# zamazincode/cv-diffusion-model

Measured on AMD Instinct MI355X. Metric: images/sec (whole node), 256×256 4-step LCM 'small'; PSNR vs CPU ref, higher is better.
Workload: dtype fp16; 1 GPU; variant=small, 256x256, batch=32/GPU, 4 LCM steps, fp16, 1xMI355X (BASELINE configs[1] per GPU); global_batch=32, parallelism=single GPU

## Files before the change

### cv-diffusion-model_amd/csrc/irbx.hip

```cpp
#include <string>
#include <type_traits>
#include <vector>

#include "common.h"
#include "kernels.h"

namespace llie {

typedef uint32_t u32x2 __attribute__((ext_vector_type(2)));

typedef __bf16 bf16x2_t __attribute__((ext_vector_type(2)));
__device__ __forceinline__ float dot2_bf16(uint32_t a, uint32_t b, float c) {
  return __builtin_amdgcn_fdot2_f32_bf16(*reinterpret_cast<const bf16x2_t*>(&a), *reinterpret_cast<const bf16x2_t*>(&b), c, false);
}

template <typename T>
__device__ __forceinline__ typename Elem<T>::vec_t activate8(typename Elem<T>::vec_t v, const float* sc, const float* sh) {
  const u32x4 x = reinterpret_cast<const u32x4&>(v);
  const f32x4 s0 = *reinterpret_cast<const f32x4*>(sc), s1 = *reinterpret_cast<const f32x4*>(sc + 4);
  const f32x4 b0 = *reinterpret_cast<const f32x4*>(sh), b1 = *reinterpret_cast<const f32x4*>(sh + 4);
  u32x4 o;
  o[0] = act_clamp01_pack<T>(x[0], s0[0], s0[1], b0[0], b0[1]);
  o[1] = act_clamp01_pack<T>(x[1], s0[2], s0[3], b0[2], b0[3]);
  o[2] = act_clamp01_pack<T>(x[2], s1[0], s1[1], b1[0], b1[1]);
// ... 102 lines not shown
      if constexpr (POOL) {
#pragma unroll
        for (int gi = 0; gi < 2; ++gi) {
          left[gi] = gcol == 0; right[gi] = gcol == w16 - 1;
          top[gi] = gidx < w16; bot[gi] = gidx >= gbot;
          edge[gi] = left[gi] || right[gi] || top[gi] || bot[gi];
          ++gidx;
          gcol = gcol + 1 == w16 ? 0 : gcol + 1;
        }
      }
#pragma unroll
      for (int j = 0; j < NBW; ++j) {
        f32x16 acc;
#pragma unroll
        for (int r = 0; r < 16; ++r) acc[r] = 0.f;
#pragma unroll
        for (int s = 0; s < KS; ++s) acc = mfma16<T>(af[s], wf[j][s], acc);
        if constexpr (STAMP) {
          asm volatile("" ::"s"(__builtin_amdgcn_readfirstlane(__float_as_int(acc[15]))));
          stamp(3);
        }
        if constexpr (POOL) {
          constexpr uint32_t ones = PackedOne<T>::lo | PackedOne<T>::hi;
          uint32_t pk[8];
#pragma unroll
          for (int i = 0; i < 8; ++i) pk[i] = affine_clamp01_pack<T>(acc[2 * i], acc[2 * i + 1], sc2[j], sc2[j], sh2[j], sh2[j]);
          float gs[2];
#pragma unroll
          for (int gi = 0; gi < 2; ++gi) {
            gs[gi] = dot2_pk<T>(pk[4 * gi], ones, 0.f);
#pragma unroll
            for (int i = 1; i < 4; ++i) gs[gi] = dot2_pk<T>(pk[4 * gi + i], ones, gs[gi]);
            if (edge[gi]) {
              asm volatile("" ::: "memory");
              const uint32_t mc0 = (left[gi] && h == 0) ? PackedOne<T>::lo : 0u;
              const uint32_t mcw = (right[gi] && h == 1) ? PackedOne<T>::hi : 0u;
              c0s[j] = dot2_pk<T>(pk[4 * gi], mc0, c0s[j]);
              cws[j] = dot2_pk<T>(pk[4 * gi + 3], mcw, cws[j]);
              if (top[gi]) {
                r0s[j] += gs[gi];
                kk[j][0] = dot2_pk<T>(pk[4 * gi], mc0, kk[j][0]);
                kk[j][1] = dot2_pk<T>(pk[4 * gi + 3], mcw, kk[j][1]);
              }
              if (bot[gi]) {
                rhs[j] += gs[gi];
                kk[j][2] = dot2_pk<T>(pk[4 * gi], mc0, kk[j][2]);
                kk[j][3] = dot2_pk<T>(pk[4 * gi + 3], mcw, kk[j][3]);
              }
            }
          }
          s1[j] += gs[0] + gs[1];
          stamp(4);
          continue;
        }
        f32x2 t1 = {0.f, 0.f}, t2 = {0.f, 0.f};
#pragma unroll
        for (int r = 0; r < 16; r += 2) {
          const f32x2 v = {acc[r], acc[r + 1]};
          t1 += v;
          t2 = __builtin_elementwise_fma(v, v, t2);
        }
        s1[j] += t1[0] + t1[1];
        s2[j] += t2[0] + t2[1];
      }
    }
  }
  if constexpr (STAMP) {
    if (a.dbg && lane == 0) {
      const size_t wg = (size_t)blockIdx.z * gridDim.x + blockIdx.x;
      for (int i = 0; i < kXStamps; ++i) a.dbg[(wg * 4 + wave) * kXStamps + i] = i < 5 ? tk[i] : 0ull;
    }
  }
  const int ntiles = P / RP;
  if constexpr (POOL) {
#pragma unroll
    for (int j = 0; j < NBW; ++j) {
      float v[9] = {s1[j], r0s[j], rhs[j], c0s[j], cws[j], kk[j][0], kk[j][1], kk[j][2], kk[j][3]};
#pragma unroll
      for (int i = 0; i < 9; ++i) v[i] += __shfl_xor(v[i], 32, 64);
      if (h == 0) {
        const int c = (wave * NBW + j) * 32 + n;
        float t = 0.f;
#pragma unroll
        for (int tap = 0; tap < 9; ++tap) {
          const int ky = tap / 3, kx = tap % 3;
          float st = v[0];
          if (ky == 2) st -= v[1];
          if (ky == 0) st -= v[2];
          if (kx == 2) st -= v[3];
          if (kx == 0) st -= v[4];
          if (ky == 2 && kx == 2) st += v[5];
          if (ky == 2 && kx == 0) st += v[6];
          if (ky == 0 && kx == 2) st += v[7];
          if (ky == 0 && kx == 0) st += v[8];
          t = __builtin_fmaf((float)(T)(6.f * a.wd[tap * a.Chid + c]), st, t);
        }
        fixed_add(a.pool_tot + (size_t)b * a.Chid + c, t, kPoolFixScale);
      }
    }
    return;
  }
#pragma unroll
  for (int j = 0; j < NBW; ++j) {
    s1[j] += __shfl_xor(s1[j], 32, 64);
    s2[j] += __shfl_xor(s2[j], 32, 64);
    if (h == 0) {
      const int c = (wave * NBW + j) * 32 + n;
      a.stats[((size_t)(b * ntiles + tile) * 2 + 0) * a.Chid + c] = 6.f * s1[j];
      a.stats[((size_t)(b * ntiles + tile) * 2 + 1) * a.Chid + c] = 36.f * s2[j];
    }
  }
}
template <int KS, int NBW>
__global__ void __launch_bounds__(256, 2) expand_pool_stamp_kernel(const IrbxArgs a, const int RP) {
  expand_scan<half_t, KS, NBW, true, true>(a, RP);
}
template <typename T, int KS, int NBW>
__global__ void __launch_bounds__(256, 2) expand_stats_kernel(const IrbxArgs a, const int RP) {
  expand_scan<T, KS, NBW, false>(a, RP);
}
template <typename T, int KS, int NBW>
__global__ void __launch_bounds__(256, 2) expand_pool_kernel(const IrbxArgs a, const int RP) {
  expand_scan<T, KS, NBW, true>(a, RP);
}

constexpr int kXT_H = 8, kXT_W = 16;
constexpr int kXH_W = kXT_W + 2, kXH_H = kXT_H + 2;
constexpr int kXNPX = kXH_W * kXH_H;
constexpr int kXNPB = 6;

constexpr int SHP = 144;

template <typename T, int KS, bool DBUF, bool STAMP, bool NTST, int PCO>
__device__ __forceinline__ void expand_dw_body(const IrbxArgs& a, const int tiles_per_wg, const int chunks_per_wg) {
  constexpr int K = 16 * KS;
  constexpr int XP = (K + 8) * 2;
  constexpr int QSTEP = 256 / (2 * KS);
  constexpr int XTHR = QSTEP * 2 * KS;
  constexpr int XPT = (kXNPX + QSTEP - 1) / QSTEP;
  constexpr int SH_BYTES = kXNPB * 32 * SHP;
  constexpr bool PREF = KS <= 2;
  typedef typename Elem<T>::vec_t vec_t;
  extern __shared__ __align__(16) unsigned char smem[];
  unsigned char* sH = smem;
  unsigned char* sX = smem + (DBUF ? 2 : 1) * SH_BYTES;
  T* wds = reinterpret_cast<T*>(sX + kXNPB * 32 * XP);
  float* aff2 = reinterpret_cast<float*>(wds + 10 * a.Chid);
  float* aff1 = aff2 + 2 * a.Chid;
  float* red = aff1 + 2 * K;
  constexpr bool PACC_LDS = KS <= 4;
  long long* pacc_lds = reinterpret_cast<long long*>(red + 2 * 256);
  long long pacc_reg[PACC_LDS ? 1 : KS];
  constexpr bool PSKIP = PCO > 0 && PCO != K;
  float* gate_s = reinterpret_cast<float*>(red + (PSKIP ? 8 * PCO : 2 * 256));
  static_assert(PCO == 0 || (!DBUF && !STAMP && (PCO == K ? PACC_LDS : PCO % 32 == 0 && PCO <= 64)),
                "project tail: single-buffered kernel; identity blocks keep the gate in the pool totals' LDS");

  const int tid = threadIdx.x, lane = tid & 63, wave = tid >> 6;
  const int n = lane & 31, h = lane >> 5;
  const int chb = wave & 1, pxg = wave >> 1;
  const int b = blockIdx.z;
  const int tiles_x = a.W / kXT_W;
  const int P = a.H * a.W;
  const T* x0 = reinterpret_cast<const T*>(a.x0) + (size_t)b * P * a.c0;
  const T* x1 = a.x1 ? reinterpret_cast<const T*>(a.x1) + (size_t)b * P * a.c1 : nullptr;
  const T* w1 = reinterpret_cast<const T*>(a.w1);
  T* out = reinterpret_cast<T*>(a.out) + (size_t)b * P * a.Chid;
  const int chunk0 = blockIdx.y * chunks_per_wg;
  const int nchunks_all = a.Chid / 64;
  const int chunk1 = chunk0 + chunks_per_wg < nchunks_all ? chunk0 + chunks_per_wg : nchunks_all;

  for (int i = tid; i < 10 * a.Chid; i += 256) {
    const int t = i & 1, c = (i >> 1) % a.Chid, tap = 2 * ((i >> 1) / a.Chid) + t;
    wds[i] = tap < 9 ? (T)(6.f * a.wd[tap * a.Chid + c]) : (T)0.f;
  }
  for (int i = tid; i < a.Chid; i += 256) {
    aff2[i] = a.as2[(size_t)b * a.Chid + i];
    aff2[a.Chid + i] = a.ab2[(size_t)b * a.Chid + i] * kSixth;
  }
  for (int i = tid; i < K; i += 256) {
    aff1[i] = a.as1[(size_t)b * K + i];
    aff1[K + i] = a.ab1[(size_t)b * K + i];
  }
  if constexpr (PCO > 0)
    for (int i = tid; i < a.Chid; i += 256) gate_s[i] = a.gate[(size_t)b * a.Chid + i];
  for (int i = tid; i < (kXNPB * 32 - kXNPX) * (XP / 16); i += 256)
    *reinterpret_cast<u32x4*>(sX + kXNPX * XP + i * 16) = u32x4{0u, 0u, 0u, 0u};

  const int ntiles_img = tiles_x * (a.H / kXT_H);
  const int tile_first = tiles_per_wg > 0 ? blockIdx.x * tiles_per_wg : (int)(blockIdx.x * (unsigned)ntiles_img / gridDim.x);
  const int tile_end = tiles_per_wg > 0 ? tile_first + tiles_per_wg : (int)((blockIdx.x + 1) * (unsigned)ntiles_img / gridDim.x);
  const int tile_last = tile_end < ntiles_img ? tile_end : ntiles_img;

  const int xkv = tid % (2 * KS), xq0 = tid / (2 * KS), xk8 = xkv * 8;
  const bool xthr = XTHR == 256 || tid < XTHR;
  const bool xseg1 = xk8 >= a.c0;
  const T* xb = xseg1 ? x1 + (xk8 - a.c0) : x0 + xk8;
  const int xc = xseg1 ? a.c1 : a.c0;
  const bool xlast = xthr && (XPT - 1) * QSTEP + xq0 < kXNPX;
  int xrel[XPT];
#pragma unroll
  for (int j = 0; j < XPT; ++j) {
    const int q = xq0 + j * QSTEP;
    xrel[j] = (q / kXH_W - 1) * a.W + (q % kXH_W - 1);
  }
  unsigned char* sxw = sX + xq0 * XP + xk8 * 2;
  vec_t raw[XPT];
  auto load_tile = [&](int ty, int tx) {
    const int pix0 = ty * kXT_H * a.W + tx * kXT_W;
    const bool border = ty == 0 || tx == 0 || ty == a.H / kXT_H - 1 || tx == tiles_x - 1;
    if (!border) {
#pragma unroll
      for (int j = 0; j < XPT; ++j) {
        if (j < XPT - 1 ? xthr : xlast) raw[j] = ld_vec<T>(xb + (size_t)(pix0 + xrel[j]) * xc);
        else raw[j] = vec_t{};
      }
    } else {
#pragma unroll
      for (int j = 0; j < XPT; ++j) {
        const int q = xq0 + j * QSTEP;
        const int gy = ty * kXT_H - 1 + q / kXH_W, gx = tx * kXT_W - 1 + q % kXH_W;
        if ((j < XPT - 1 ? xthr : xlast) && gy >= 0 && gy < a.H && gx >= 0 && gx < a.W) raw[j] = ld_vec<T>(xb + (size_t)(pix0 + xrel[j]) * xc);
        else raw[j] = vec_t{};
      }
    }
  };
  int ty = tile_first / tiles_x, tx = tile_first % tiles_x;
  if (PREF && tile_first < tile_last) load_tile(ty, tx);
  vec_t wf[KS];
  auto load_wf = [&](int chunk) {
#pragma unroll
    for (int s = 0; s < KS; ++s) wf[s] = ld_vec<T>(w1 + (size_t)(chunk * 64 + chb * 32 + n) * K + 16 * s + 8 * h);
  };
  load_wf(chunk0);
  wg_barrier();

  unsigned long long tk[kXStamps] = {}, t_prev = 0;
  auto stamp = [&](int slot) {
    if constexpr (STAMP) {
      __builtin_amdgcn_sched_barrier(0);
      const unsigned long long now = __builtin_amdgcn_s_memtime();
      __builtin_amdgcn_sched_barrier(0);
      if (slot >= 0) tk[slot] += now - t_prev;
      t_prev = now;
    }
  };
  stamp(-1);
  const bool has_pool = PCO == 0 && (a.pool != nullptr || a.pool_tot != nullptr);
  int par = 0;
  int pend_tile = -1, pend_chunk = 0, pend_par = 0;
  if constexpr (PCO > 0) {
  } else if constexpr (PACC_LDS) {
    if (tid < 64) {
#pragma unroll
      for (int q = 0; q < KS; ++q) pacc_lds[q * 64 + tid] = 0;
    }
  } else {
#pragma unroll
    for (int q = 0; q < KS; ++q) pacc_reg[q] = 0;
  }
  auto flush_pool = [&]() {
    if constexpr (PCO > 0) {
      if (pend_tile >= 0 && tid < 2 * PCO) {
        const float t = (red[tid] + red[2 * PCO + tid]) + (red[4 * PCO + tid] + red[6 * PCO + tid]);
        a.ystats[((size_t)b * ntiles_img + pend_tile) * 2 * PCO + tid] = t;
      }
      pend_tile = -1;
      return;
    }
    if (pend_tile >= 0 && tid < 64) {
      const float* r = red + pend_par * 256;
      const int cbb = tid >> 5, ci = tid & 31;
      const float t = r[cbb * 64 + ci] + r[(cbb + 2) * 64 + ci];
      if (a.pool_tot) {
        const long long v = __float2ll_rn(t * kPoolFixScale);
        if constexpr (PACC_LDS) {
          pacc_lds[(pend_chunk - chunk0) * 64 + tid] += v;
        } else {
#pragma unroll
          for (int q = 0; q < KS; ++q) pacc_reg[q] += (pend_chunk - chunk0 == q) ? v : 0ll;
        }
      } else {
        a.pool[((size_t)b * ntiles_img + pend_tile) * a.Chid + pend_chunk * 64 + tid] = t;
      }
    }
    pend_tile = -1;
  };

  for (int tile = tile_first; tile < tile_last; ++tile) {
    const int y0 = ty * kXT_H, x0p = tx * kXT_W;
    int tyn = ty, txn = tx + 1;
    if (txn == tiles_x) { txn = 0; ++tyn; }
    if (!PREF) load_tile(ty, tx);
    __builtin_amdgcn_s_waitcnt(0x0F70);
    stamp(0);
#pragma unroll
    for (int j = 0; j < XPT; ++j) {
      if (j < XPT - 1 ? xthr : xlast)
        *reinterpret_cast<vec_t*>(sxw + j * QSTEP * XP) = activate8<T>(raw[j], aff1 + xk8, aff1 + K + xk8);
    }
    stamp(1);
    if (PREF && tile + 1 < tile_last) load_tile(tyn, txn);
    const bool border = ty == 0 || tx == 0 || ty == a.H / kXT_H - 1 || tx == tiles_x - 1;
    bool ok[3] = {true, true, true};
    if (border) {
#pragma unroll
      for (int i = 0; i < 3; ++i) {
        const int q = (pxg * 3 + i) * 32 + n;
        const int gy = y0 - 1 + q / kXH_W, gx = x0p - 1 + q % kXH_W;
        ok[i] = q < kXNPX && gy >= 0 && gy < a.H && gx >= 0 && gx < a.W;
      }
    }
    stamp(2);
    wg_barrier();
    stamp(3);
    if (!DBUF) flush_pool();
    stamp(4);

    typedef float f32x4v __attribute__((ext_vector_type(4)));
    constexpr int NCB = PCO > 0 ? PCO / 16 : 1;
    f32x4v yacc[2][NCB];
#pragma unroll
    for (int r = 0; r < 2; ++r)
#pragma unroll
      for (int cb = 0; cb < NCB; ++cb) yacc[r][cb] = f32x4v{0.f, 0.f, 0.f, 0.f};
    for (int chunk = chunk0; chunk < chunk1; ++chunk) {
      unsigned char* buf = sH + (DBUF ? par * SH_BYTES : 0);
      if (!DBUF && chunk > chunk0) {
        wg_barrier();
        flush_pool();
        stamp(5);
      }
      const int ch0 = chunk * 64 + chb * 32;
      f32x4 sc2[4], sh2[4];
#pragma unroll
      for (int g = 0; g < 4; ++g) {
        sc2[g] = *reinterpret_cast<const f32x4*>(aff2 + ch0 + 8 * g + 4 * h);
        sh2[g] = *reinterpret_cast<const f32x4*>(aff2 + a.Chid + ch0 + 8 * g + 4 * h);
      }
      constexpr int NACC = (KS <= 2 && PCO == 0) ? 3 : 1;
      f32x16 accs[NACC];
      if constexpr (NACC == 3) {
#pragma unroll
        for (int i = 0; i < 3; ++i) {
          const int q = (pxg * 3 + i) * 32 + n;
#pragma unroll
          for (int r = 0; r < 16; ++r) accs[i][r] = 0.f;
#pragma unroll
          for (int s = 0; s < KS; ++s)
            accs[i] = mfma16<T>(wf[s], *reinterpret_cast<const vec_t*>(sX + q * XP + (16 * s + 8 * h) * 2), accs[i]);
        }
        load_wf(chunk + 1 < chunk1 ? chunk + 1 : chunk0);
      }
#pragma unroll
      for (int i = 0; i < 3; ++i) {
        const int q = (pxg * 3 + i) * 32 + n;
        if constexpr (NACC == 1) {
#pragma unroll
          for (int r = 0; r < 16; ++r) accs[0][r] = 0.f;
#pragma unroll
          for (int s = 0; s < KS; ++s)
            accs[0] = mfma16<T>(wf[s], *reinterpret_cast<const vec_t*>(sX + q * XP + (16 * s + 8 * h) * 2), accs[0]);
          if (i == 2) load_wf(chunk + 1 < chunk1 ? chunk + 1 : chunk0);
        }
        const f32x16 acc = accs[NACC == 3 ? i : 0];
        uint32_t pk[4][2];
#pragma unroll
        for (int g = 0; g < 4; ++g)
#pragma unroll
          for (int j = 0; j < 2; ++j)
            pk[g][j] = affine_clamp01_pack<T>(acc[4 * g + 2 * j], acc[4 * g + 2 * j + 1], sc2[g][2 * j], sc2[g][2 * j + 1],
                                              sh2[g][2 * j], sh2[g][2 * j + 1]);
        if (border) {
#pragma unroll
          for (int g = 0; g < 4; ++g)
#pragma unroll
            for (int j = 0; j < 2; ++j) pk[g][j] = ok[i] ? pk[g][j] : 0u;
        }
        u32x4 lo, hi2;
#pragma unroll
        for (int j = 0; j < 2; ++j) {
          const u32x2 r02 = __builtin_amdgcn_permlane32_swap(pk[0][j], pk[2][j], false, false);
          const u32x2 r13 = __builtin_amdgcn_permlane32_swap(pk[1][j], pk[3][j], false, false);
          lo[j] = r02[0]; lo[2 + j] = r02[1];
          hi2[j] = r13[0]; hi2[2 + j] = r13[1];
        }
        *reinterpret_cast<u32x4*>(buf + q * SHP + (chb * 4 + 2 * h) * 16) = lo;
        *reinterpret_cast<u32x4*>(buf + q * SHP + (chb * 4 + 2 * h + 1) * 16) = hi2;
      }
      stamp(6);
      wg_barrier();
      if (DBUF) flush_pool();
      stamp(7);
      if constexpr (PCO > 0) {
        const int li = lane & 15, g = lane >> 4;
        uint32_t amask[4];
#pragma unroll
        for (int d = 0; d < 4; ++d)
          amask[d] = (((li & 7) >> 1) == d && (g >> 1) == (li >> 3)) ? ((li & 1) ? 0xFFFF0000u : 0x0000FFFFu) : 0u;
        const uint32_t* wpair = reinterpret_cast<const uint32_t*>(wds) + chunk * 64 + li;
        const uint32_t wsel = (g & 1) ? 0x03020302u : 0x01000100u;
        const int choff = 8 * (g >> 1) + 16 * (g & 1);
        vec_t wpf[NCB][2];
        const T* wp = reinterpret_cast<const T*>(a.wp) + (size_t)li * a.ldp + chunk * 64 + choff;
#pragma unroll
        for (int cb = 0; cb < NCB; ++cb)
#pragma unroll
          for (int kb = 0; kb < 2; ++kb) wpf[cb][kb] = ld_vec<T>(wp + (size_t)cb * 16 * a.ldp + 32 * kb);
        f32x4v dacc[4][2];
#pragma unroll
        for (int c = 0; c < 4; ++c)
#pragma unroll
          for (int r = 0; r < 2; ++r) dacc[c][r] = f32x4v{0.f, 0.f, 0.f, 0.f};
        const unsigned char* bbase = buf + ((2 * wave) * kXH_W + li) * SHP + (g >> 1) * 16;
        const bool upper = (g & 1) != 0;
        vec_t bf[2][2];
        uint32_t wq[2];
        auto ld_step = [&](int step, vec_t (&bb)[2], uint32_t& w2) {
          const int pr = step >> 2, c = step & 3;
          const int ta = 2 * pr, tb = 2 * pr + 1 < 9 ? 2 * pr + 1 : 8;
          const int offa = (ta / 3) * kXH_W + ta % 3, offb = (tb / 3) * kXH_W + tb % 3;
          const unsigned char* p0 = bbase + (upper ? offb : offa) * SHP + c * 32;
#pragma unroll
          for (int r = 0; r < 2; ++r) bb[r] = *reinterpret_cast<const vec_t*>(p0 + r * kXH_W * SHP);
          w2 = wpair[pr * a.Chid + 16 * c];
        };
        ld_step(0, bf[0], wq[0]);
#pragma unroll
        for (int step = 0; step < 20; ++step) {
          if (step + 1 < 20) ld_step(step + 1, bf[(step + 1) & 1], wq[(step + 1) & 1]);
          __builtin_amdgcn_sched_barrier(0);
          const int c = step & 3;
          const uint32_t wdup = __builtin_amdgcn_perm(wq[step & 1], wq[step & 1], wsel);
          u32x4 t;
#pragma unroll
          for (int d = 0; d < 4; ++d) t[d] = wdup & amask[d];
          const vec_t af = reinterpret_cast<const vec_t&>(t);
#pragma unroll
          for (int r = 0; r < 2; ++r) dacc[c][r] = mfma16x16<T>(af, bf[step & 1][r], dacc[c][r]);
        }
#pragma unroll
        for (int c = 0; c < 4; ++c) {
          const f32x4 gt = *reinterpret_cast<const f32x4*>(gate_s + chunk * 64 + 16 * c + 4 * g);
#pragma unroll
          for (int r = 0; r < 2; ++r)
#pragma unroll
            for (int e = 0; e < 4; ++e) dacc[c][r][e] *= gt[e];
        }
#pragma unroll
        for (int r = 0; r < 2; ++r)
#pragma unroll
          for (int kb = 0; kb < 2; ++kb) {
            uint32_t p0[2], p1[2];
#pragma unroll
            for (int j = 0; j < 2; ++j) {
              typedef T t2 __attribute__((ext_vector_type(2)));
              t2 o0, o1;
              o0[0] = (T)dacc[2 * kb][r][2 * j]; o0[1] = (T)dacc[2 * kb][r][2 * j + 1];
              o1[0] = (T)dacc[2 * kb + 1][r][2 * j]; o1[1] = (T)dacc[2 * kb + 1][r][2 * j + 1];
              p0[j] = *reinterpret_cast<uint32_t*>(&o0);
              p1[j] = *reinterpret_cast<uint32_t*>(&o1);
            }
            const u32x2 s0 = __builtin_amdgcn_permlane16_swap(p0[0], p1[0], false, false);
            const u32x2 s1 = __builtin_amdgcn_permlane16_swap(p0[1], p1[1], false, false);
            const u32x4 v = {s0[0], s1[0], s0[1], s1[1]};
#pragma unroll
            for (int cb = 0; cb < NCB; ++cb) yacc[r][cb] = mfma16x16<T>(wpf[cb][kb], reinterpret_cast<const vec_t&>(v), yacc[r][cb]);
          }
      } else {
        const int li = lane & 15, g = lane >> 4;
        uint32_t amask[4];
#pragma unroll
        for (int d = 0; d < 4; ++d)
          amask[d] = (((li & 7) >> 1) == d && (g >> 1) == (li >> 3)) ? ((li & 1) ? 0xFFFF0000u : 0x0000FFFFu) : 0u;
        const uint32_t* wpair = reinterpret_cast<const uint32_t*>(wds) + chunk * 64 + chb * 32 + li;
        const uint32_t wsel = (g & 1) ? 0x03020302u : 0x01000100u;
        f32x4v dacc[2][4];
#pragma unroll
        for (int c2 = 0; c2 < 2; ++c2)
#pragma unroll
          for (int r = 0; r < 4; ++r) dacc[c2][r] = f32x4v{0.f, 0.f, 0.f, 0.f};
        const unsigned char* bbase = buf + ((4 * pxg) * kXH_W + li) * SHP + (chb * 4 + (g >> 1)) * 16;
        const bool upper = (g & 1) != 0;
        vec_t bf[2][4];
        uint32_t wq[2];
        auto ld_step = [&](int step, vec_t (&bb)[4], uint32_t& w2) {
          const int pr = step >> 1, c2 = step & 1;
          const int ta = 2 * pr, tb = 2 * pr + 1 < 9 ? 2 * pr + 1 : 8;
          const int offa = (ta / 3) * kXH_W + ta % 3, offb = (tb / 3) * kXH_W + tb % 3;
          const unsigned char* p0 = bbase + (upper ? offb : offa) * SHP + c2 * 32;
#pragma unroll
          for (int r = 0; r < 4; ++r) bb[r] = *reinterpret_cast<const vec_t*>(p0 + r * kXH_W * SHP);
          w2 = wpair[pr * a.Chid + 16 * c2];
        };
        ld_step(0, bf[0], wq[0]);
#pragma unroll
        for (int step = 0; step < 10; ++step) {
          if (step + 1 < 10) ld_step(step + 1, bf[(step + 1) & 1], wq[(step + 1) & 1]);
          __builtin_amdgcn_sched_barrier(0);
          const int c2 = step & 1;
          const uint32_t wdup = __builtin_amdgcn_perm(wq[step & 1], wq[step & 1], wsel);
          u32x4 t;
#pragma unroll
          for (int d = 0; d < 4; ++d) t[d] = wdup & amask[d];
          const vec_t af = reinterpret_cast<const vec_t&>(t);
#pragma unroll
          for (int r = 0; r < 4; ++r) dacc[c2][r] = mfma16x16<T>(af, bf[step & 1][r], dacc[c2][r]);
        }
        const int choff = 8 * (g >> 1) + 16 * (g & 1);
#pragma unroll
        for (int r = 0; r < 4; ++r) {
          uint32_t p0[2], p1[2];
#pragma unroll
          for (int j = 0; j < 2; ++j) {
            typedef T t2 __attribute__((ext_vector_type(2)));
            t2 o0, o1;
            o0[0] = (T)dacc[0][r][2 * j]; o0[1] = (T)dacc[0][r][2 * j + 1];
            o1[0] = (T)dacc[1][r][2 * j]; o1[1] = (T)dacc[1][r][2 * j + 1];
            p0[j] = *reinterpret_cast<uint32_t*>(&o0);
            p1[j] = *reinterpret_cast<uint32_t*>(&o1);
          }
          const u32x2 s0 = __builtin_amdgcn_permlane16_swap(p0[0], p1[0], false, false);
          const u32x2 s1 = __builtin_amdgcn_permlane16_swap(p0[1], p1[1], false, false);
          const u32x4 v = {s0[0], s1[0], s0[1], s1[1]};
          const int orow = 4 * pxg + r;
          T* op = out + ((size_t)(y0 + orow) * a.W + x0p + li) * a.Chid + chunk * 64 + chb * 32 + choff;
          if constexpr (NTST) __builtin_nontemporal_store(v, reinterpret_cast<u32x4*>(op));
          else *reinterpret_cast<u32x4*>(op) = v;
        }
        if (has_pool) {
          float v[8];
#pragma unroll
          for (int c2 = 0; c2 < 2; ++c2)
#pragma unroll
            for (int e = 0; e < 4; ++e) v[4 * c2 + e] = (dacc[c2][0][e] + dacc[c2][1][e]) + (dacc[c2][2][e] + dacc[c2][3][e]);
#define LLIE_DPP_STEP(ROR)                                                                                               \
  _Pragma("unroll") for (int i = 0; i < 8; ++i)                                                                          \
      asm volatile("v_add_f32_dpp %0, %0, %0 row_ror:" #ROR " row_mask:0xf bank_mask:0xf" : "+v"(v[i]));
          asm volatile("s_nop 1" : "+v"(v[0]), "+v"(v[1]), "+v"(v[2]), "+v"(v[3]), "+v"(v[4]), "+v"(v[5]), "+v"(v[6]), "+v"(v[7]));
          LLIE_DPP_STEP(8)
          LLIE_DPP_STEP(4)
          LLIE_DPP_STEP(2)
          LLIE_DPP_STEP(1)
#undef LLIE_DPP_STEP
          if (li == 0) {
            float* rp = red + (DBUF ? par : 0) * 256 + wave * 64 + 4 * g;
            *reinterpret_cast<f32x4*>(rp) = f32x4{v[0], v[1], v[2], v[3]};
            *reinterpret_cast<f32x4*>(rp + 16) = f32x4{v[4], v[5], v[6], v[7]};
          }
          pend_tile = tile; pend_chunk = chunk; pend_par = DBUF ? par : 0;
        }
      }
      if (DBUF) par ^= 1;
      stamp(8);
    }
    if constexpr (PCO > 0) {
      const int li = lane & 15, g = lane >> 4;
      const int choff = 8 * (g >> 1) + 16 * (g & 1);
      T* yout = reinterpret_cast<T*>(a.y) + (size_t)b * P * PCO;
      if constexpr (PSKIP) {
        const T* wsk = reinterpret_cast<const T*>(a.wp) + (size_t)li * a.ldp + a.Chid + 8 * g;
#pragma unroll
        for (int ks = 0; ks < K / 32; ++ks) {
          const int ch = 32 * ks + 8 * g;
          vec_t wsf[NCB];
#pragma unroll
          for (int cb = 0; cb < NCB; ++cb) wsf[cb] = ld_vec<T>(wsk + (size_t)cb * 16 * a.ldp + 32 * ks);
#pragma unroll
          for (int r = 0; r < 2; ++r) {
            const size_t pix = (size_t)(y0 + 2 * wave + r) * a.W + x0p + li;
            const vec_t xv = ch < a.c0 ? ld_vec<T>(x0 + pix * a.c0 + ch) : ld_vec<T>(x1 + pix * a.c1 + (ch - a.c0));
#pragma unroll
            for (int cb = 0; cb < NCB; ++cb) yacc[r][cb] = mfma16x16<T>(wsf[cb], xv, yacc[r][cb]);
          }
        }
      }
      float st[2][NCB * 4];
#pragma unroll
      for (int i = 0; i < NCB * 4; ++i) st[0][i] = st[1][i] = 0.f;
#pragma unroll
      for (int r = 0; r < 2; ++r) {
        const size_t pix = (size_t)(y0 + 2 * wave + r) * a.W + x0p + li;
        uint32_t pk[NCB][2];
#pragma unroll
        for (int cb = 0; cb < NCB; ++cb) {
          typedef T t4 __attribute__((ext_vector_type(4)));
          typedef T t2 __attribute__((ext_vector_type(2)));
          t4 res = t4{};
          if constexpr (!PSKIP) res = *reinterpret_cast<const t4*>(x0 + pix * PCO + 16 * cb + 4 * g);
#pragma unroll
          for (int j = 0; j < 2; ++j) {
            t2 o;
#pragma unroll
            for (int e = 0; e < 2; ++e) {
              o[e] = PSKIP ? (T)yacc[r][cb][2 * j + e] : (T)(yacc[r][cb][2 * j + e] + (float)res[2 * j + e]);
              const float q = (float)o[e];
              st[0][4 * cb + 2 * j + e] += q;
              st[1][4 * cb + 2 * j + e] = __builtin_fmaf(q, q, st[1][4 * cb + 2 * j + e]);
            }
            pk[cb][j] = *reinterpret_cast<uint32_t*>(&o);
          }
        }
#pragma unroll
        for (int pp = 0; pp < NCB / 2; ++pp) {
          const u32x2 s0 = __builtin_amdgcn_permlane16_swap(pk[2 * pp][0], pk[2 * pp + 1][0], false, false);
          const u32x2 s1 = __builtin_amdgcn_permlane16_swap(pk[2 * pp][1], pk[2 * pp + 1][1], false, false);
          *reinterpret_cast<u32x4*>(yout + pix * PCO + 32 * pp + choff) = u32x4{s0[0], s1[0], s0[1], s1[1]};
        }
      }
#pragma unroll
      for (int w8 = 0; w8 < NCB; ++w8) {
        float* v = &st[w8 & 1][(w8 >> 1) * 8];
#define LLIE_DPP_STEP(ROR)                                                                                               \
  _Pragma("unroll") for (int i = 0; i < 8; ++i)                                                                          \
      asm volatile("v_add_f32_dpp %0, %0, %0 row_ror:" #ROR " row_mask:0xf bank_mask:0xf" : "+v"(v[i]));
        asm volatile("s_nop 1" : "+v"(v[0]), "+v"(v[1]), "+v"(v[2]), "+v"(v[3]), "+v"(v[4]), "+v"(v[5]), "+v"(v[6]), "+v"(v[7]));
        LLIE_DPP_STEP(8)
        LLIE_DPP_STEP(4)
        LLIE_DPP_STEP(2)
        LLIE_DPP_STEP(1)
#undef LLIE_DPP_STEP
      }
      if (li == 0) {
#pragma unroll
        for (int which = 0; which < 2; ++which)
#pragma unroll
          for (int cb = 0; cb < NCB; ++cb)
            *reinterpret_cast<f32x4*>(red + (wave * 2 + which) * PCO + 16 * cb + 4 * g) =
                f32x4{st[which][4 * cb], st[which][4 * cb + 1], st[which][4 * cb + 2], st[which][4 * cb + 3]};
      }
      pend_tile = tile;
    }
    ty = tyn; tx = txn;
  }
  if constexpr (STAMP) {
    if (a.dbg && lane == 0) {
      const size_t wg = ((size_t)blockIdx.z * gridDim.y + blockIdx.y) * gridDim.x + blockIdx.x;
#pragma unroll
      for (int i = 0; i < kXStamps; ++i) a.dbg[(wg * 4 + wave) * kXStamps + i] = tk[i];
    }
  }
  if constexpr (PCO > 0) {
    wg_barrier();
    flush_pool();
  }
  if (has_pool) {
    wg_barrier();
    flush_pool();
    if (a.pool_tot && tid < 64) {
#pragma unroll
      for (int q = 0; q < KS; ++q)
        if (chunk0 + q < chunk1) atomicAdd(a.pool_tot + (size_t)b * a.Chid + (chunk0 + q) * 64 + tid, (unsigned long long)(PACC_LDS ? pacc_lds[q * 64 + tid] : pacc_reg[PACC_LDS ? 0 : q]));
    }
  }
}

template <typename T, int KS, bool DBUF, bool STAMP = false, bool NTST = false>
__global__ void __launch_bounds__(256, (KS == 2 && !DBUF) ? 3 : 2) expand_dw_kernel(const IrbxArgs a, const int tiles_per_wg, const int chunks_per_wg) {
  expand_dw_body<T, KS, DBUF, STAMP, NTST, 0>(a, tiles_per_wg, chunks_per_wg);
}
template <typename T, int KS, int PCO>
__global__ void __launch_bounds__(256, KS == 2 ? 3 : 2) expand_dw_project_kernel(const IrbxArgs a, const int tiles_per_wg) {
  expand_dw_body<T, KS, false, false, false, PCO>(a, tiles_per_wg, KS);
}

bool irbx_supported(int dtype, int Cin, int c0, int Chid, int H, int W) {
  if (dtype != 1 && dtype != 2) return false;
  if (Cin != 32 && Cin != 64 && Cin != 96) return false;
  if (c0 % 16 || Chid != 4 * Cin) return false;
  return W % kXT_W == 0 && H % kXT_H == 0 && (H * W) % irbx_stats_rows(H * W) == 0;
}
int irbx_pool_tiles(int H, int W) { return (H / kXT_H) * (W / kXT_W); }
int irbx_project_supported(int dtype, int Cin, int c0, int Chid, int Cout, bool skip, int H, int W) {
  if (!irbx_supported(dtype, Cin, c0, Chid, H, W)) return 0;
  if (!skip) return (Cin == 32 || Cin == 64) && Cout == Cin && c0 == Cin ? kIrbxProjectIdentity : 0;
  return Cin == 96 && Cout == 32 ? kIrbxProjectSkip : 0;
}
int irbx_project_tiles(int H, int W) { return irbx_pool_tiles(H, W); }
int irbx_stats_rows(int P) {
  int rp = 128;
  while (rp < 1024 && rp * 2 * 64 <= P) rp *= 2;
  return rp;
}

static int g_irbx_dbuf = 0, g_irbx_stamp = 0;
static int g_irbx_grid[3] = {0, 0, 0};
void irbx_grid(int ks, int v) {
  for (int i = 0; i < 3; ++i)
    if (ks == 0 || ks == 2 * (i + 1)) g_irbx_grid[i] = v;
}
static unsigned long long* g_irbx_dbg = nullptr;
static size_t g_irbx_dbg_n = 0;
void irbx_stamp(int v) { g_irbx_stamp = v; }
hipError_t irbx_stamp_fetch(double* out) {
  if (!g_irbx_dbg || !g_irbx_dbg_n) return hipErrorInvalidValue;
  std::vector<unsigned long long> h(g_irbx_dbg_n);
  hipError_t e = hipMemcpy(h.data(), g_irbx_dbg, g_irbx_dbg_n * 8, hipMemcpyDeviceToHost);
  if (e != hipSuccess) return e;
  for (int i = 0; i < kXStamps; ++i) out[i] = 0.0;
  for (size_t i = 0; i < g_irbx_dbg_n; ++i) out[i % kXStamps] += (double)h[i];
  for (int i = 0; i < kXStamps; ++i) out[i] /= (double)(g_irbx_dbg_n / kXStamps);
  out[kXStamps] = (double)(g_irbx_dbg_n / kXStamps);
  return hipSuccess;
}
void irbx_tune(int dbuf) { if (dbuf >= 0) g_irbx_dbuf = dbuf; }

template <typename T, int KS, int NBW, bool POOL>
static hipError_t launch_scan_cfg(const IrbxArgs& a, hipStream_t s) {
  const int P = a.H * a.W, RP = irbx_stats_rows(P);
  static const std::string name = std::string(POOL ? "expand_pool_kernel<" : "expand_stats_kernel<") + TypeName<T>::value + ", " +
                                  std::to_string(KS) + ", " + std::to_string(NBW) + ">";
  note_kernel(name.c_str());
  if constexpr (POOL && std::is_same<T, half_t>::value) {
    if (g_irbx_stamp == 2) {
      IrbxArgs b = a;
      const size_t n = (size_t)(P / RP) * a.B * 4 * kXStamps;
      if (n > g_irbx_dbg_n || !g_irbx_dbg) {
        if (g_irbx_dbg) (void)hipFree(g_irbx_dbg);
        hipError_t e = hipMalloc(reinterpret_cast<void**>(&g_irbx_dbg), n * 8);
        if (e != hipSuccess) return e;
      }
      g_irbx_dbg_n = n;
      b.dbg = g_irbx_dbg;
      hipLaunchKernelGGL((expand_pool_stamp_kernel<KS, NBW>), dim3(P / RP, 1, a.B), dim3(256), 0, s, b, RP);
      return hipGetLastError();
    }
  }
  constexpr auto kernel = POOL ? &expand_pool_kernel<T, KS, NBW> : &expand_stats_kernel<T, KS, NBW>;
  hipLaunchKernelGGL(kernel, dim3(P / RP, 1, a.B), dim3(256), 0, s, a, RP);
  return hipGetLastError();
}
template <typename T, bool POOL>
static hipError_t launch_scan_t(const IrbxArgs& a, hipStream_t s) {
  switch (a.c0 + a.c1) {
    case 32: return launch_scan_cfg<T, 2, 1, POOL>(a, s);
    case 64: return launch_scan_cfg<T, 4, 2, POOL>(a, s);
    case 96: return launch_scan_cfg<T, 6, 3, POOL>(a, s);
  }
  return hipErrorInvalidValue;
}
hipError_t launch_expand_stats(int dtype, const IrbxArgs& a, hipStream_t s) {
  if (!irbx_supported(dtype, a.c0 + a.c1, a.c0, a.Chid, a.H, a.W) || (a.c1 && !a.x1) || !a.stats) return hipErrorInvalidValue;
  return dtype == 1 ? launch_scan_t<half_t, false>(a, s) : launch_scan_t<bf16_t, false>(a, s);
}
hipError_t launch_expand_pool(int dtype, const IrbxArgs& a, hipStream_t s) {
  if (!irbx_supported(dtype, a.c0 + a.c1, a.c0, a.Chid, a.H, a.W) || (a.c1 && !a.x1) || !a.pool_tot || !a.as2 || !a.ab2 || !a.wd)
    return hipErrorInvalidValue;
  return dtype == 1 ? launch_scan_t<half_t, true>(a, s) : launch_scan_t<bf16_t, true>(a, s);
}

constexpr size_t irbx_lds_bytes(int KS, int Chid, bool dbuf, int PCO) {
  const size_t body = (size_t)(dbuf ? 2 : 1) * kXNPB * 32 * SHP + (size_t)kXNPB * 32 * (16 * KS + 8) * 2 + (size_t)10 * Chid * 2 +
                      (size_t)2 * Chid * 4 + (size_t)2 * 16 * KS * 4;
  if (PCO != 0 && PCO != 16 * KS) return body + (size_t)8 * PCO * 4 + (size_t)Chid * 4;
  return body + 2 * 256 * 4 + (KS <= 4 ? (size_t)KS * 64 * 8 : 0);
}
static_assert(irbx_lds_bytes(6, 384, false, 32) == 81664 && irbx_lds_bytes(6, 384, false, 32) <= 80 * 1024, "expand_dw_project<6, 32>: two workgroups per CU");

constexpr int kXTilesPerWg = 4;
static int irbx_tiles_per_wg(const IrbxArgs& a) {
  int tpw = kXTilesPerWg;
  while (tpw > 1 && ((a.W / kXT_W) % tpw || (long)(irbx_pool_tiles(a.H, a.W) / tpw) * a.B < 2048)) tpw >>= 1;
  return tpw;
}

template <typename T, int KS, bool DBUF, bool STAMP, bool NTST>
static hipError_t launch_dw_one(const IrbxArgs& a, dim3 grid, size_t lds, int tpw, int cpw, hipStream_t s) {
  static std::atomic<uint64_t> attr_done{0};
  if (hipError_t e = ensure_max_lds(reinterpret_cast<const void*>(&expand_dw_kernel<T, KS, DBUF, STAMP, NTST>), 128 * 1024, attr_done); e != hipSuccess)
    return e;
  hipLaunchKernelGGL((expand_dw_kernel<T, KS, DBUF, STAMP, NTST>), grid, dim3(256), lds, s, a, tpw, cpw);
  return hipGetLastError();
}
template <typename T, int KS, bool DBUF>
static hipError_t launch_dw_cfg(const IrbxArgs& a, hipStream_t s) {
  const size_t lds = irbx_lds_bytes(KS, a.Chid, DBUF, 0);
  const int ntiles = irbx_pool_tiles(a.H, a.W), nchunks = a.Chid / 64;
  int tpw = irbx_tiles_per_wg(a);
  int cpw = nchunks;
  while (cpw > 1 && (long)(ntiles / tpw) * a.B * (nchunks / cpw) < 1024 && cpw % 2 == 0) cpw >>= 1;
  static const std::string name = std::string("expand_dw_kernel<") + TypeName<T>::value + ", " + std::to_string(KS) + ", " +
                                  (DBUF ? "1" : "0") + ">";
  note_kernel(name.c_str());
  dim3 grid(ntiles / tpw, nchunks / cpw, a.B);
  if (g_irbx_grid[KS / 2 - 1] > 0) {
    int gx = g_irbx_grid[KS / 2 - 1] / (a.B * (nchunks / cpw));
    gx = gx < 1 ? 1 : (gx > ntiles ? ntiles : gx);
    grid.x = gx;
    tpw = 0;
  }
  if constexpr (std::is_same<T, half_t>::value && !DBUF) {
    if (g_irbx_stamp == 1) {
      IrbxArgs b = a;
      const size_t n = (size_t)grid.x * grid.y * grid.z * 4 * kXStamps;
      if (n > g_irbx_dbg_n || !g_irbx_dbg) {
        if (g_irbx_dbg) (void)hipFree(g_irbx_dbg);
        hipError_t e = hipMalloc(reinterpret_cast<void**>(&g_irbx_dbg), n * 8);
        if (e != hipSuccess) return e;
      }
      g_irbx_dbg_n = n;
      b.dbg = g_irbx_dbg;
      return launch_dw_one<T, KS, DBUF, true, false>(b, grid, lds, tpw, cpw, s);
    }
  }
  if constexpr (!DBUF) {
    if (a.nt) return launch_dw_one<T, KS, DBUF, false, true>(a, grid, lds, tpw, cpw, s);
  }
  return launch_dw_one<T, KS, DBUF, false, false>(a, grid, lds, tpw, cpw, s);
}
template <typename T>
static hipError_t launch_dw_t(const IrbxArgs& a, hipStream_t s) {
  const int Cin = a.c0 + a.c1;
  switch (Cin) {
    case 32: return g_irbx_dbuf ? launch_dw_cfg<T, 2, true>(a, s) : launch_dw_cfg<T, 2, false>(a, s);
    case 64: return launch_dw_cfg<T, 4, false>(a, s);
    case 96: return launch_dw_cfg<T, 6, false>(a, s);
  }
  return hipErrorInvalidValue;
}
template <typename T, int KS, int PCO>
static hipError_t launch_project_cfg(const IrbxArgs& a, hipStream_t s) {
  const size_t lds = irbx_lds_bytes(KS, a.Chid, false, PCO);
  const int ntiles = irbx_pool_tiles(a.H, a.W), tpw = irbx_tiles_per_wg(a);
  static const std::string name = std::string("expand_dw_project_kernel<") + TypeName<T>::value + ", " + std::to_string(KS) +
                                  (PCO == 16 * KS ? std::string() : ", " + std::to_string(PCO)) + ">";
  note_kernel(name.c_str());
  static std::atomic<uint64_t> attr_done{0};
  if (hipError_t e = ensure_max_lds(reinterpret_cast<const void*>(&expand_dw_project_kernel<T, KS, PCO>), 128 * 1024, attr_done); e != hipSuccess) return e;
  hipLaunchKernelGGL((expand_dw_project_kernel<T, KS, PCO>), dim3(ntiles / tpw, 1, a.B), dim3(256), lds, s, a, tpw);
  return hipGetLastError();
}
template <typename T>
static hipError_t launch_project_t(const IrbxArgs& a, int form, hipStream_t s) {
  if (form == kIrbxProjectSkip) return launch_project_cfg<T, 6, 32>(a, s);
  return a.c0 == 32 ? launch_project_cfg<T, 2, 32>(a, s) : launch_project_cfg<T, 4, 64>(a, s);
}
hipError_t launch_expand_dw_project(int dtype, const IrbxArgs& a0, int cout, bool skip, hipStream_t s) {
  IrbxArgs a = a0;
  const int Cin = a.c0 + a.c1;
  if (!skip) a.ldp = a.Chid;
  const int form = irbx_project_supported(dtype, Cin, a.c0, a.Chid, cout, skip, a.H, a.W);
  if (!form || (a.c1 != 0) != (a.x1 != nullptr) || a.ldp < a.Chid + (skip ? Cin : 0) || a.ldp % 8 || !a.gate || !a.wp || !a.y || !a.ystats ||
      !a.as2 || !a.ab2 || !a.wd)
    return hipErrorInvalidValue;
  return dtype == 1 ? launch_project_t<half_t>(a, form, s) : launch_project_t<bf16_t>(a, form, s);
}
hipError_t launch_expand_dw(int dtype, const IrbxArgs& a, hipStream_t s) {
  if (!irbx_supported(dtype, a.c0 + a.c1, a.c0, a.Chid, a.H, a.W) || (a.c1 && !a.x1) || !a.out) return hipErrorInvalidValue;
  return dtype == 1 ? launch_dw_t<half_t>(a, s) : launch_dw_t<bf16_t>(a, s);
}

}
```

Measured before the change: 1126 images/sec.

## Fold gate into depthwise weights, hoist residual/skip loads, widen DPP stats reduction

For project-tail kernels (except KS=4), the per-channel gate is folded into the depthwise weights when they are staged into LDS. This drops the per-chunk gate multiply and the gate LDS array, shrinking LDS. The residual and skip-path loads, plus the skip MFMAs, move ahead of the chunk loop so their latency overlaps the tile prefetch and barrier, at the cost of extra live registers. The statistics reduction now combines 16 values per DPP tree with mirror and halve steps, and a stamp-instrumented project kernel variant is added for timing.

New measurement: 1140 images/sec (median of 6 runs). +1.3%, better.

```diff
diff --git a/cv-diffusion-model_amd/csrc/irbx.hip b/cv-diffusion-model_amd/csrc/irbx.hip
--- a/cv-diffusion-model_amd/csrc/irbx.hip
+++ b/cv-diffusion-model_amd/csrc/irbx.hip
@@ -278,9 +278,10 @@
   long long* pacc_lds = reinterpret_cast<long long*>(red + 2 * 256);
   long long pacc_reg[PACC_LDS ? 1 : KS];
   constexpr bool PSKIP = PCO > 0 && PCO != K;
-  float* gate_s = reinterpret_cast<float*>(red + (PSKIP ? 8 * PCO : 2 * 256));
-  static_assert(PCO == 0 || (!DBUF && !STAMP && (PCO == K ? PACC_LDS : PCO % 32 == 0 && PCO <= 64)),
-                "project tail: single-buffered kernel; identity blocks keep the gate in the pool totals' LDS");
+  constexpr bool GATEW = PCO > 0 && KS != 4;
+  float* gate_s = red + 8 * PCO;
+  static_assert(PCO == 0 || (!DBUF && (PCO == K ? KS <= 4 : PCO % 32 == 0 && PCO <= 64)),
+                "project tail: single-buffered kernel; identity form at 32 and 64 channels, skip form to 32 or 64");
 
   const int tid = threadIdx.x, lane = tid & 63, wave = tid >> 6;
   const int n = lane & 31, h = lane >> 5;
@@ -298,7 +299,8 @@
 
   for (int i = tid; i < 10 * a.Chid; i += 256) {
     const int t = i & 1, c = (i >> 1) % a.Chid, tap = 2 * ((i >> 1) / a.Chid) + t;
-    wds[i] = tap < 9 ? (T)(6.f * a.wd[tap * a.Chid + c]) : (T)0.f;
+    if constexpr (GATEW) wds[i] = tap < 9 ? (T)(6.f * a.wd[tap * a.Chid + c] * a.gate[(size_t)b * a.Chid + c]) : (T)0.f;
+    else wds[i] = tap < 9 ? (T)(6.f * a.wd[tap * a.Chid + c]) : (T)0.f;
   }
   for (int i = tid; i < a.Chid; i += 256) {
     aff2[i] = a.as2[(size_t)b * a.Chid + i];
@@ -308,7 +310,7 @@
     aff1[i] = a.as1[(size_t)b * K + i];
     aff1[K + i] = a.ab1[(size_t)b * K + i];
   }
-  if constexpr (PCO > 0)
+  if constexpr (PCO > 0 && !GATEW)
     for (int i = tid; i < a.Chid; i += 256) gate_s[i] = a.gate[(size_t)b * a.Chid + i];
   for (int i = tid; i < (kXNPB * 32 - kXNPX) * (XP / 16); i += 256)
     *reinterpret_cast<u32x4*>(sX + kXNPX * XP + i * 16) = u32x4{0u, 0u, 0u, 0u};
@@ -362,7 +364,7 @@
   wg_barrier();
 
   unsigned long long tk[kXStamps] = {}, t_prev = 0;
-  auto stamp = [&](int slot) {
+  auto stamp_at = [&](int slot) {
     if constexpr (STAMP) {
       __builtin_amdgcn_sched_barrier(0);
       const unsigned long long now = __builtin_amdgcn_s_memtime();
@@ -371,7 +373,9 @@
       t_prev = now;
     }
   };
-  stamp(-1);
+  auto stamp = [&](int slot) { if constexpr (PCO == 0) stamp_at(slot); };
+  auto pstamp = [&](int slot) { if constexpr (PCO > 0) stamp_at(slot); };
+  stamp_at(-1);
   const bool has_pool = PCO == 0 && (a.pool != nullptr || a.pool_tot != nullptr);
   int par = 0;
   int pend_tile = -1, pend_chunk = 0, pend_par = 0;
@@ -420,12 +424,42 @@
     if (!PREF) load_tile(ty, tx);
     __builtin_amdgcn_s_waitcnt(0x0F70);
     stamp(0);
+    pstamp(0);
 #pragma unroll
     for (int j = 0; j < XPT; ++j) {
       if (j < XPT - 1 ? xthr : xlast)
         *reinterpret_cast<vec_t*>(sxw + j * QSTEP * XP) = activate8<T>(raw[j], aff1 + xk8, aff1 + K + xk8);
     }
     stamp(1);
+    constexpr int NCB = PCO > 0 ? PCO / 16 : 1;
+    constexpr int NKS = PSKIP ? K / 32 : 1;
+    typedef T t4 __attribute__((ext_vector_type(4)));
+    t4 res[2][NCB];
+    vec_t wsf[NKS][NCB], xsv[NKS][2];
+    if constexpr (PCO > 0) {
+      const int li = lane & 15, g = lane >> 4;
+#pragma unroll
+      for (int r = 0; r < 2; ++r) {
+        const size_t pix = (size_t)(y0 + 2 * wave + r) * a.W + x0p + li;
+        if constexpr (!PSKIP) {
+#pragma unroll
+          for (int cb = 0; cb < NCB; ++cb) res[r][cb] = *reinterpret_cast<const t4*>(x0 + pix * PCO + 16 * cb + 4 * g);
+        } else {
+#pragma unroll
+          for (int ks = 0; ks < NKS; ++ks) {
+            const int ch = 32 * ks + 8 * g;
+            xsv[ks][r] = ch < a.c0 ? ld_vec<T>(x0 + pix * a.c0 + ch) : ld_vec<T>(x1 + pix * a.c1 + (ch - a.c0));
+          }
+        }
+      }
+      if constexpr (PSKIP) {
+        const T* wsk = reinterpret_cast<const T*>(a.wp) + (size_t)li * a.ldp + a.Chid + 8 * g;
+#pragma unroll
+        for (int ks = 0; ks < NKS; ++ks)
+#pragma unroll
+          for (int cb = 0; cb < NCB; ++cb) wsf[ks][cb] = ld_vec<T>(wsk + (size_t)cb * 16 * a.ldp + 32 * ks);
+      }
+    }
     if (PREF && tile + 1 < tile_last) load_tile(tyn, txn);
     const bool border = ty == 0 || tx == 0 || ty == a.H / kXT_H - 1 || tx == tiles_x - 1;
     bool ok[3] = {true, true, true};
@@ -438,24 +472,37 @@
       }
     }
     stamp(2);
+    pstamp(1);
     wg_barrier();
     stamp(3);
     if (!DBUF) flush_pool();
     stamp(4);
 
     typedef float f32x4v __attribute__((ext_vector_type(4)));
-    constexpr int NCB = PCO > 0 ? PCO / 16 : 1;
     f32x4v yacc[2][NCB];
 #pragma unroll
     for (int r = 0; r < 2; ++r)
 #pragma unroll
-      for (int cb = 0; cb < NCB; ++cb) yacc[r][cb] = f32x4v{0.f, 0.f, 0.f, 0.f};
+      for (int cb = 0; cb < NCB; ++cb) {
+        if constexpr (PCO > 0 && !PSKIP) yacc[r][cb] = f32x4v{(float)res[r][cb][0], (float)res[r][cb][1], (float)res[r][cb][2], (float)res[r][cb][3]};
+        else yacc[r][cb] = f32x4v{0.f, 0.f, 0.f, 0.f};
+      }
+    if constexpr (PSKIP) {
+#pragma unroll
+      for (int ks = 0; ks < NKS; ++ks)
+#pragma unroll
+        for (int r = 0; r < 2; ++r)
+#pragma unroll
+          for (int cb = 0; cb < NCB; ++cb) yacc[r][cb] = mfma16x16<T>(wsf[ks][cb], xsv[ks][r], yacc[r][cb]);
+    }
+    pstamp(2);
     for (int chunk = chunk0; chunk < chunk1; ++chunk) {
       unsigned char* buf = sH + (DBUF ? par * SH_BYTES : 0);
       if (!DBUF && chunk > chunk0) {
         wg_barrier();
         flush_pool();
         stamp(5);
+        pstamp(3);
       }
       const int ch0 = chunk * 64 + chb * 32;
       f32x4 sc2[4], sh2[4];
@@ -515,9 +562,11 @@
         *reinterpret_cast<u32x4*>(buf + q * SHP + (chb * 4 + 2 * h + 1) * 16) = hi2;
       }
       stamp(6);
+      pstamp(4);
       wg_barrier();
       if (DBUF) flush_pool();
       stamp(7);
+      pstamp(5);
       if constexpr (PCO > 0) {
         const int li = lane & 15, g = lane >> 4;
         uint32_t amask[4];
@@ -565,13 +614,19 @@
 #pragma unroll
           for (int r = 0; r < 2; ++r) dacc[c][r] = mfma16x16<T>(af, bf[step & 1][r], dacc[c][r]);
         }
-#pragma unroll
-        for (int c = 0; c < 4; ++c) {
-          const f32x4 gt = *reinterpret_cast<const f32x4*>(gate_s + chunk * 64 + 16 * c + 4 * g);
-#pragma unroll
-          for (int r = 0; r < 2; ++r)
-#pragma unroll
-            for (int e = 0; e < 4; ++e) dacc[c][r][e] *= gt[e];
+        if constexpr (STAMP) {
+          asm volatile("" ::"s"(__builtin_amdgcn_readfirstlane(__float_as_int(dacc[3][1][3]))));
+          pstamp(6);
+        }
+        if constexpr (!GATEW) {
+#pragma unroll
+          for (int c = 0; c < 4; ++c) {
+            const f32x4 gt = *reinterpret_cast<const f32x4*>(gate_s + chunk * 64 + 16 * c + 4 * g);
+#pragma unroll
+            for (int r = 0; r < 2; ++r)
+#pragma unroll
+              for (int e = 0; e < 4; ++e) dacc[c][r][e] *= gt[e];
+          }
         }
 #pragma unroll
         for (int r = 0; r < 2; ++r)
@@ -593,6 +648,7 @@
 #pragma unroll
             for (int cb = 0; cb < NCB; ++cb) yacc[r][cb] = mfma16x16<T>(wpf[cb][kb], reinterpret_cast<const vec_t&>(v), yacc[r][cb]);
           }
+        pstamp(7);
       } else {
         const int li = lane & 15, g = lane >> 4;
         uint32_t amask[4];
@@ -684,23 +740,6 @@
       const int li = lane & 15, g = lane >> 4;
       const int choff = 8 * (g >> 1) + 16 * (g & 1);
       T* yout = reinterpret_cast<T*>(a.y) + (size_t)b * P * PCO;
-      if constexpr (PSKIP) {
-        const T* wsk = reinterpret_cast<const T*>(a.wp) + (size_t)li * a.ldp + a.Chid + 8 * g;
-#pragma unroll
-        for (int ks = 0; ks < K / 32; ++ks) {
-          const int ch = 32 * ks + 8 * g;
-          vec_t wsf[NCB];
-#pragma unroll
-          for (int cb = 0; cb < NCB; ++cb) wsf[cb] = ld_vec<T>(wsk + (size_t)cb * 16 * a.ldp + 32 * ks);
-#pragma unroll
-          for (int r = 0; r < 2; ++r) {
-            const size_t pix = (size_t)(y0 + 2 * wave + r) * a.W + x0p + li;
-            const vec_t xv = ch < a.c0 ? ld_vec<T>(x0 + pix * a.c0 + ch) : ld_vec<T>(x1 + pix * a.c1 + (ch - a.c0));
-#pragma unroll
-            for (int cb = 0; cb < NCB; ++cb) yacc[r][cb] = mfma16x16<T>(wsf[cb], xv, yacc[r][cb]);
-          }
-        }
-      }
       float st[2][NCB * 4];
 #pragma unroll
       for (int i = 0; i < NCB * 4; ++i) st[0][i] = st[1][i] = 0.f;
@@ -710,16 +749,13 @@
         uint32_t pk[NCB][2];
 #pragma unroll
         for (int cb = 0; cb < NCB; ++cb) {
-          typedef T t4 __attribute__((ext_vector_type(4)));
           typedef T t2 __attribute__((ext_vector_type(2)));
-          t4 res = t4{};
-          if constexpr (!PSKIP) res = *reinterpret_cast<const t4*>(x0 + pix * PCO + 16 * cb + 4 * g);
 #pragma unroll
           for (int j = 0; j < 2; ++j) {
             t2 o;
 #pragma unroll
             for (int e = 0; e < 2; ++e) {
-              o[e] = PSKIP ? (T)yacc[r][cb][2 * j + e] : (T)(yacc[r][cb][2 * j + e] + (float)res[2 * j + e]);
+              o[e] = (T)yacc[r][cb][2 * j + e];
               const float q = (float)o[e];
               st[0][4 * cb + 2 * j + e] += q;
               st[1][4 * cb + 2 * j + e] = __builtin_fmaf(q, q, st[1][4 * cb + 2 * j + e]);
@@ -735,27 +771,37 @@
         }
       }
 #pragma unroll
-      for (int w8 = 0; w8 < NCB; ++w8) {
-        float* v = &st[w8 & 1][(w8 >> 1) * 8];
-#define LLIE_DPP_STEP(ROR)                                                                                               \
-  _Pragma("unroll") for (int i = 0; i < 8; ++i)                                                                          \
-      asm volatile("v_add_f32_dpp %0, %0, %0 row_ror:" #ROR " row_mask:0xf bank_mask:0xf" : "+v"(v[i]));
-        asm volatile("s_nop 1" : "+v"(v[0]), "+v"(v[1]), "+v"(v[2]), "+v"(v[3]), "+v"(v[4]), "+v"(v[5]), "+v"(v[6]), "+v"(v[7]));
-        LLIE_DPP_STEP(8)
-        LLIE_DPP_STEP(4)
-        LLIE_DPP_STEP(2)
-        LLIE_DPP_STEP(1)
+      for (int grp = 0; grp < NCB / 2; ++grp) {
+        float v[16];
+#pragma unroll
+        for (int j = 0; j < 16; ++j) {
+          if constexpr (NCB == 2) v[j] = st[j >> 3][j & 7];
+          else v[j] = st[grp][j];
+        }
+        asm volatile("s_nop 1" : "+v"(v[0]), "+v"(v[1]), "+v"(v[2]), "+v"(v[3]), "+v"(v[4]), "+v"(v[5]), "+v"(v[6]), "+v"(v[7]),
+                                 "+v"(v[8]), "+v"(v[9]), "+v"(v[10]), "+v"(v[11]), "+v"(v[12]), "+v"(v[13]), "+v"(v[14]), "+v"(v[15]));
+#define LLIE_DPP_HALVE(N, CTRL, KEEP, TAKE)                                                                                  \
+  _Pragma("unroll") for (int i = 0; i < N; ++i)                                                                              \
+      asm volatile("v_add_f32_dpp %0, %0, %0 " CTRL " row_mask:0xf bank_mask:" KEEP : "+v"(v[i]));                           \
+  _Pragma("unroll") for (int i = 0; i < N; ++i)                                                                              \
+      asm volatile("v_add_f32_dpp %0, %1, %1 " CTRL " row_mask:0xf bank_mask:" TAKE : "+v"(v[i]) : "v"(v[i + N]));
+#define LLIE_DPP_STEP(CTRL)                                                                                                  \
+  _Pragma("unroll") for (int i = 0; i < 4; ++i)                                                                              \
+      asm volatile("v_add_f32_dpp %0, %0, %0 " CTRL " row_mask:0xf bank_mask:0xf" : "+v"(v[i]));
+        LLIE_DPP_HALVE(8, "row_mirror", "0x3", "0xc")
+        LLIE_DPP_HALVE(4, "row_half_mirror", "0x5", "0xa")
+        LLIE_DPP_STEP("quad_perm:[2,3,0,1]")
+        LLIE_DPP_STEP("quad_perm:[1,0,3,2]")
+#undef LLIE_DPP_HALVE
 #undef LLIE_DPP_STEP
-      }
-      if (li == 0) {
-#pragma unroll
-        for (int which = 0; which < 2; ++which)
-#pragma unroll
-          for (int cb = 0; cb < NCB; ++cb)
-            *reinterpret_cast<f32x4*>(red + (wave * 2 + which) * PCO + 16 * cb + 4 * g) =
-                f32x4{st[which][4 * cb], st[which][4 * cb + 1], st[which][4 * cb + 2], st[which][4 * cb + 3]};
+        if ((li & 3) == 0) {
+          const int k = li >> 2;
+          const int which = NCB == 2 ? k >> 1 : grp, cb = NCB == 2 ? k & 1 : k;
+          *reinterpret_cast<f32x4*>(red + (wave * 2 + which) * PCO + 16 * cb + 4 * g) = f32x4{v[0], v[1], v[2], v[3]};
+        }
       }
       pend_tile = tile;
+      pstamp(8);
     }
     ty = tyn; tx = txn;
   }
@@ -788,6 +834,10 @@
 template <typename T, int KS, int PCO>
 __global__ void __launch_bounds__(256, KS == 2 ? 3 : 2) expand_dw_project_kernel(const IrbxArgs a, const int tiles_per_wg) {
   expand_dw_body<T, KS, false, false, false, PCO>(a, tiles_per_wg, KS);
+}
+template <int KS, int PCO>
+__global__ void __launch_bounds__(256, KS == 2 ? 3 : 2) expand_dw_project_stamp_kernel(const IrbxArgs a, const int tiles_per_wg) {
+  expand_dw_body<half_t, KS, false, true, false, PCO>(a, tiles_per_wg, KS);
 }
 
 bool irbx_supported(int dtype, int Cin, int c0, int Chid, int H, int W) {
@@ -830,6 +880,18 @@
   return hipSuccess;
 }
 void irbx_tune(int dbuf) { if (dbuf >= 0) g_irbx_dbuf = dbuf; }
+static hipError_t irbx_dbg_buffer(size_t waves, IrbxArgs& a) {
+  const size_t n = waves * kXStamps;
+  if (n > g_irbx_dbg_n || !g_irbx_dbg) {
+    if (g_irbx_dbg) (void)hipFree(g_irbx_dbg);
+    g_irbx_dbg = nullptr;
+    hipError_t e = hipMalloc(reinterpret_cast<void**>(&g_irbx_dbg), n * 8);
+    if (e != hipSuccess) return e;
+  }
+  g_irbx_dbg_n = n;
+  a.dbg = g_irbx_dbg;
+  return hipSuccess;
+}
 
 template <typename T, int KS, int NBW, bool POOL>
 static hipError_t launch_scan_cfg(const IrbxArgs& a, hipStream_t s) {
@@ -840,14 +902,7 @@
   if constexpr (POOL && std::is_same<T, half_t>::value) {
     if (g_irbx_stamp == 2) {
       IrbxArgs b = a;
-      const size_t n = (size_t)(P / RP) * a.B * 4 * kXStamps;
-      if (n > g_irbx_dbg_n || !g_irbx_dbg) {
-        if (g_irbx_dbg) (void)hipFree(g_irbx_dbg);
-        hipError_t e = hipMalloc(reinterpret_cast<void**>(&g_irbx_dbg), n * 8);
-        if (e != hipSuccess) return e;
-      }
-      g_irbx_dbg_n = n;
-      b.dbg = g_irbx_dbg;
+      if (hipError_t e = irbx_dbg_buffer((size_t)(P / RP) * a.B * 4, b); e != hipSuccess) return e;
       hipLaunchKernelGGL((expand_pool_stamp_kernel<KS, NBW>), dim3(P / RP, 1, a.B), dim3(256), 0, s, b, RP);
       return hipGetLastError();
     }
@@ -878,10 +933,10 @@
 constexpr size_t irbx_lds_bytes(int KS, int Chid, bool dbuf, int PCO) {
   const size_t body = (size_t)(dbuf ? 2 : 1) * kXNPB * 32 * SHP + (size_t)kXNPB * 32 * (16 * KS + 8) * 2 + (size_t)10 * Chid * 2 +
                       (size_t)2 * Chid * 4 + (size_t)2 * 16 * KS * 4;
-  if (PCO != 0 && PCO != 16 * KS) return body + (size_t)8 * PCO * 4 + (size_t)Chid * 4;
+  if (PCO != 0) return body + (size_t)8 * PCO * 4 + (KS == 4 ? (size_t)Chid * 4 : 0);
   return body + 2 * 256 * 4 + (KS <= 4 ? (size_t)KS * 64 * 8 : 0);
 }
-static_assert(irbx_lds_bytes(6, 384, false, 32) == 81664 && irbx_lds_bytes(6, 384, false, 32) <= 80 * 1024, "expand_dw_project<6, 32>: two workgroups per CU");
+static_assert(irbx_lds_bytes(6, 384, false, 32) == 80128 && irbx_lds_bytes(6, 384, false, 32) <= 80 * 1024, "expand_dw_project<6, 32>: two workgroups per CU");
 
 constexpr int kXTilesPerWg = 4;
 static int irbx_tiles_per_wg(const IrbxArgs& a) {
@@ -918,14 +973,7 @@
   if constexpr (std::is_same<T, half_t>::value && !DBUF) {
     if (g_irbx_stamp == 1) {
       IrbxArgs b = a;
-      const size_t n = (size_t)grid.x * grid.y * grid.z * 4 * kXStamps;
-      if (n > g_irbx_dbg_n || !g_irbx_dbg) {
-        if (g_irbx_dbg) (void)hipFree(g_irbx_dbg);
-        hipError_t e = hipMalloc(reinterpret_cast<void**>(&g_irbx_dbg), n * 8);
-        if (e != hipSuccess) return e;
-      }
-      g_irbx_dbg_n = n;
-      b.dbg = g_irbx_dbg;
+      if (hipError_t e = irbx_dbg_buffer((size_t)grid.x * grid.y * grid.z * 4, b); e != hipSuccess) return e;
       return launch_dw_one<T, KS, DBUF, true, false>(b, grid, lds, tpw, cpw, s);
     }
   }
@@ -951,6 +999,17 @@
   static const std::string name = std::string("expand_dw_project_kernel<") + TypeName<T>::value + ", " + std::to_string(KS) +
                                   (PCO == 16 * KS ? std::string() : ", " + std::to_string(PCO)) + ">";
   note_kernel(name.c_str());
+  if constexpr (std::is_same<T, half_t>::value) {
+    if (g_irbx_stamp == 3) {
+      IrbxArgs b = a;
+      if (hipError_t e = irbx_dbg_buffer((size_t)(ntiles / tpw) * a.B * 4, b); e != hipSuccess) return e;
+      static std::atomic<uint64_t> stamp_attr_done{0};
+      if (hipError_t e = ensure_max_lds(reinterpret_cast<const void*>(&expand_dw_project_stamp_kernel<KS, PCO>), 128 * 1024, stamp_attr_done); e != hipSuccess)
+        return e;
+      hipLaunchKernelGGL((expand_dw_project_stamp_kernel<KS, PCO>), dim3(ntiles / tpw, 1, a.B), dim3(256), lds, s, b, tpw);
+      return hipGetLastError();
+    }
+  }
   static std::atomic<uint64_t> attr_done{0};
   if (hipError_t e = ensure_max_lds(reinterpret_cast<const void*>(&expand_dw_project_kernel<T, KS, PCO>), 128 * 1024, attr_done); e != hipSuccess) return e;
   hipLaunchKernelGGL((expand_dw_project_kernel<T, KS, PCO>), dim3(ntiles / tpw, 1, a.B), dim3(256), lds, s, a, tpw);
```
